# probabilists/zuko

Hardware: AMD Instinct MI355X
Metric: log_prob samples/sec, NSF d=64 K=8 bins=8 batch=2^20 (higher is better)
Workload: dtype f32; 1 GPU; NSF(features=64, context=0, transforms=8, bins=8, hidden=[256]*3) log_prob, batch=2^20 per GPU, x~N(0,1), seed-0 init; batch_per_gpu=1048576, global_batch=1048576, parallelism=batch-sharded x1, one RCCL all-reduce of the scalar NLL

## Files before the change

### zuko_amd/csrc/fused_ar_half_impl.h

```cpp
#pragma once
#include "fused_ar_split_impl.h"

#ifndef ARH_LOOK
#define ARH_LOOK 1
#endif
#ifndef ARH_RELU_INT
#define ARH_RELU_INT 0
#endif
#ifndef ARH_EPI_PINNED
#define ARH_EPI_PINNED 1
#endif
#ifndef ARH_DESCALE_PK
#define ARH_DESCALE_PK 1
#endif
#ifndef ARH_PREFETCH
#define ARH_PREFETCH 1
#endif

namespace zk {

typedef _Float16 f16x8 __attribute__((ext_vector_type(8)));

struct ArhB {
  f16x8 h, l;
};

__device__ __forceinline__ void arh_scale(float& amax, float& s, float& inv_s) {
  amax = fmaxf(amax, __shfl_xor(amax, 16, 64));
  amax = fmaxf(amax, __shfl_xor(amax, 32, 64));
  int e = __builtin_amdgcn_frexp_expf(amax);
  int ea = 15 - e;
  ea = ea > 90 ? 90 : (ea < -90 ? -90 : ea);
  s = __builtin_amdgcn_ldexpf(1.0f, ea);
  inv_s = __builtin_amdgcn_ldexpf(1.0f, -ea);
}

#define ARH_AMAX_OVERFLOW (65520.f * 0x1p90f)

typedef unsigned arh_u32x4 __attribute__((ext_vector_type(4)));
typedef float arh_f32x2 __attribute__((ext_vector_type(2)));

__device__ __forceinline__ void arh_split(const f32x4& lo, const f32x4& hi, float s, ArhB& b) {
  if (ARX_ABL == 6) {
    b.h = __builtin_bit_cast(f16x8, lo); b.l = __builtin_bit_cast(f16x8, hi);
    return;
  }
#if ARH_EPI_PINNED
  const float nz = -0.f;
  arh_u32x4 h, l;
#pragma unroll
  for (int e = 0; e < 4; ++e) asm("v_fma_mixlo_f16 %0, %1, %2, %3" : "=v"(h[e]) : "v"(e < 2 ? lo[2 * e] : hi[2 * e - 4]), "v"(s), "s"(nz));
#pragma unroll
  for (int e = 0; e < 4; ++e) asm("v_fma_mixhi_f16 %0, %1, %2, %3" : "+v"(h[e]) : "v"(e < 2 ? lo[2 * e + 1] : hi[2 * e - 3]), "v"(s), "s"(nz));
#pragma unroll
  for (int e = 0; e < 4; ++e) asm("v_fma_mixlo_f16 %0, %1, %2, -%3 op_sel:[0,0,0] op_sel_hi:[0,0,1]" : "=v"(l[e]) : "v"(e < 2 ? lo[2 * e] : hi[2 * e - 4]), "v"(s), "v"(h[e]));
#pragma unroll
  for (int e = 0; e < 4; ++e) asm("v_fma_mixhi_f16 %0, %1, %2, -%3 op_sel:[0,0,1] op_sel_hi:[0,0,1]" : "+v"(l[e]) : "v"(e < 2 ? lo[2 * e + 1] : hi[2 * e - 3]), "v"(s), "v"(h[e]));
  b.h = __builtin_bit_cast(f16x8, h); b.l = __builtin_bit_cast(f16x8, l);
  return;
#endif
#pragma unroll
  for (int e = 0; e < 8; ++e) {
    const float v = (e < 4 ? lo[e] : hi[e - 4]) * s;
    const _Float16 h = (_Float16)v;
    const float r = v - (float)h;
    b.h[e] = h;
    b.l[e] = (_Float16)r;
  }
}

#define ARH_MFMA(A, B, C) C = __builtin_amdgcn_mfma_f32_16x16x32_f16(__builtin_bit_cast(f16x8, A), B, C, 0, 0, 0)
__device__ __forceinline__ void arh_block(const f32x4 (&a)[2], const ArhB& b, f32x4& c) {
  if (ARX_ABL == 2) {
    asm volatile("" ::"v"(a[0]), "v"(a[1]));
    return;
  }
  ARH_MFMA(a[1], b.h, c);
  ARH_MFMA(a[0], b.l, c);
  ARH_MFMA(a[0], b.h, c);
}

__device__ __forceinline__ void arh_touch(f32x4& v) { asm volatile("" : "+v"(v)); }
template <int N> __device__ __forceinline__ void arh_settle(f32x4& a0, f32x4& a1) { asm volatile("s_waitcnt lgkmcnt(%2)" : "+v"(a0), "+v"(a1) : "n"(N)); }
template <int N> __device__ __forceinline__ void arh_settle(f32x4& a0, f32x4& a1, f32x4& a2) { asm volatile("s_waitcnt lgkmcnt(%3)" : "+v"(a0), "+v"(a1), "+v"(a2) : "n"(N)); }

template <int WAVES, int CH, int NR> struct ArhRing : ArRingS<WAVES, CH, NR> {
  typedef ArRingS<WAVES, CH, NR> B;
  template <int XV> __device__ __forceinline__ void advance_x() {
    asm volatile("s_waitcnt vmcnt(%0) lgkmcnt(0)" ::"n"((NR - 2) * B::PER + XV) : "memory");
    if (ARX_ABL != 4) __builtin_amdgcn_s_barrier();
    asm volatile("" ::: "memory");
    this->issue();
    this->slot = (this->slot + 1 == NR) ? 0 : this->slot + 1;
    this->cur_off = this->lds_off + (unsigned)(this->slot * CH * AR_TF * 4 + this->lane * 16);
  }
  template <int S, int XV = 0> __device__ __forceinline__ f32x4 read() {
    if constexpr (XV != 0 && S % CH == 0) {
      advance_x<XV>();
      f32x4 v;
      if (ARX_ABL == 5) {
        asm volatile("v_mov_b32 %0, %1" : "=v"(v[0]) : "v"(this->cur_off));
        v[1] = v[2] = v[3] = v[0];
        return v;
      }
      asm volatile("ds_read_b128 %0, %1 offset:%2" : "=v"(v) : "v"(this->cur_off), "n"((S % CH) * AR_TF * 4));
      return v;
    } else {
      return B::template read<S>();
    }
  }
};

template <int WAVES, int CH, int IMAGES, int BPOS, bool FLOW = false> struct ArhRing4 {
  static constexpr int NR = 4, PER = CH / WAVES, PIVOT = PER > 4 ? 4 : 0, CHB = CH * AR_TF * 4, NCH = (IMAGES + CH - 1) / CH;
  static_assert(PER * WAVES == CH && PER <= 6 && BPOS % 2 == 0 && BPOS >= 2 * (ARH_LOOK + 1) && BPOS + 1 < CH && CH % 2 == 0 && IMAGES % 2 == 0, "ring geometry");
  static constexpr int trigger(int c) {
    const int last = (IMAGES < (c + 1) * CH ? IMAGES : (c + 1) * CH) - 1;
    return c * CH + BPOS + 1 < last ? c * CH + BPOS + 1 : last;
  }
  static constexpr int first_trigger_from(int pos) {
    for (int c = 0; c < NCH; ++c)
      if (trigger(c) >= pos) return trigger(c);
    return -1;
  }
  const char* gsrc;
  char* ldst;
  unsigned goff, gend;
  unsigned fill_off;
  unsigned read_off;
  unsigned lane_off;
  unsigned lane16;
  unsigned cur_off;
  bool rows_in_flight;
  const char* bias_src;
  char* bias_dst;
  int bias_n, wave_id;
  __device__ __forceinline__ void bias_request() {
    for (int p = wave_id; p < bias_n; p += WAVES)
      __builtin_amdgcn_global_load_lds((const __attribute__((address_space(1))) void*)(bias_src + p * 1024 + (size_t)lane16), (__attribute__((address_space(3))) void*)(bias_dst + p * 1024), 16, 0, 0);
  }
  __device__ __forceinline__ void start(float* lds, const float* stream, int n_chunks, int wave, int lane) {
    const int b0 = wave * PER + PIVOT;
    gsrc = reinterpret_cast<const char*>(stream + b0 * AR_TF);
    ldst = reinterpret_cast<char*>(lds + b0 * AR_TF);
    goff = 0; gend = (unsigned)n_chunks * CHB; fill_off = 0;
    lane16 = (unsigned)lane * 16;
    lane_off = (unsigned)(size_t)((__attribute__((address_space(3))) float*)lds) + lane16;
    if constexpr (FLOW) { wave_id = wave; rows_in_flight = false; bias_n = 0; }
#pragma unroll
    for (int i = 0; i < NR - 1; ++i) issue();
    read_off = (NR - 1) * CHB;
    cur_off = lane_off;
  }
  template <int I> __device__ __forceinline__ void dma(const char* g, char* l) {
    if constexpr (I < PER) {
      __builtin_amdgcn_global_load_lds((const __attribute__((address_space(1))) void*)g, (__attribute__((address_space(3))) void*)l, 16, (I - PIVOT) * AR_TF * 4, 0);
      dma<I + 1>(g, l);
    }
  }
  __device__ __forceinline__ void issue() {
    asm volatile("" : "+v"(lane16));
    if (ARX_ABL != 1) dma<0>(gsrc + goff + (size_t)lane16, ldst + fill_off);
    goff = (goff + CHB == gend) ? 0 : goff + CHB;
    fill_off = (fill_off + CHB == NR * CHB) ? 0 : fill_off + CHB;
  }
  template <int XV, bool DRAIN> __device__ __forceinline__ void wait() {
    if constexpr (DRAIN) asm volatile("s_waitcnt vmcnt(%0) lgkmcnt(0)" ::"n"(XV) : "memory");
    else asm volatile("s_waitcnt vmcnt(%0)" ::"n"(XV) : "memory");
  }
  template <int XV, bool DRAIN> __device__ __forceinline__ void boundary() {
    if constexpr (FLOW && XV != 0) {
      if (rows_in_flight) wait<XV, DRAIN>();
      else wait<0, DRAIN>();
    } else {
      wait<XV, DRAIN>();
    }
    if (ARX_ABL != 4) __builtin_amdgcn_s_barrier();
    asm volatile("" ::: "memory");
    issue();
    asm volatile("" ::: "memory");
  }
  template <int S, int XV = 0> __device__ __forceinline__ f32x4 read() {
    static_assert(S >= 0 && S < IMAGES, "stream position");
    if constexpr (S % CH == 0) {
      read_off = (read_off + CHB == NR * CHB) ? 0 : read_off + CHB;
      cur_off = lane_off + read_off;
    }
    f32x4 v;
    if (ARX_ABL == 5) {
      asm volatile("v_mov_b32 %0, %1" : "=v"(v[0]) : "v"(cur_off));
      v[1] = v[2] = v[3] = v[0];
    } else {
      asm volatile("ds_read_b128 %0, %1 offset:%2" : "=v"(v) : "v"(cur_off), "n"((S % CH) * AR_TF * 4));
    }
    if constexpr (S == trigger(S / CH)) boundary<XV, (S % CH != BPOS + 1)>();
    if constexpr (FLOW && NCH >= 2) {
      if constexpr (S == trigger(NCH - 2)) bias_request();
    }
    return v;
  }
};

template <class S, int L, bool ALT> constexpr int arh_ip(int s) {
  if constexpr (ALT) return S::B_IP_ALT[s];
  else return ArxPat<S>::ip(L, s);
}
template <class S, int L, class Ring, bool ALT = false> __device__ __forceinline__ void arh_hidden(Ring& ring, const float* bias_q, const ArhB (&in)[S::TMAX / 2], f32x4 (&out)[S::TMAX], float d) {
  typedef ArxPat<S> P;
  constexpr int NB = S::NB[L], BASE = S::BASE[L], HTL = S::HT[L];
  ars_for<HTL>([&](auto t_) ARS_ALWAYS_INLINE {
    constexpr int t = t_;
    if constexpr (!P::tile_has_blocks(L, t)) out[t] = *reinterpret_cast<const f32x4*>(bias_q + t * 16);
  });
  if constexpr (NB > 0) {
    constexpr int LOOK = ARH_LOOK < NB ? ARH_LOOK : NB;
    f32x4 a[LOOK + 1][2];
    f32x4 bs;
    f32x4 acc;
    const unsigned bias_addr = arx_lds_addr(bias_q);
    ars_for<LOOK>([&](auto b_) ARS_ALWAYS_INLINE {
      constexpr int b = b_;
      ars_for<2>([&](auto p) ARS_ALWAYS_INLINE { a[b][p] = ring.template read<BASE + 2 * b + decltype(p)::value>(); });
    });
    ars_for<NB>([&](auto s_) ARS_ALWAYS_INLINE {
      constexpr int s = s_, ot = P::ot(L, s), cur = s % (LOOK + 1);
      constexpr int ip = arh_ip<S, L, ALT>(s);
      constexpr bool first_of_tile = (s == 0 || P::ot(L, s - 1) != ot), last_of_tile = (s + 1 == NB || P::ot(L, s + 1) != ot);
      if constexpr (first_of_tile) acc = f32x4{0.f, 0.f, 0.f, 0.f};
      if constexpr (last_of_tile) bs = arx_lds_raw<ot * 64>(bias_addr);
      if constexpr (s + LOOK < NB) {
        constexpr int nx = (s + LOOK) % (LOOK + 1);
        ars_for<2>([&](auto p) ARS_ALWAYS_INLINE { a[nx][p] = ring.template read<BASE + 2 * (s + LOOK) + decltype(p)::value>(); });
      }
      constexpr int ahead = (s + LOOK < NB ? LOOK : NB - 1 - s);
      if constexpr (last_of_tile) arh_settle<(s + LOOK < NB ? 2 : 0)>(a[cur][0], a[cur][1], bs);
      else arh_settle<2 * ahead>(a[cur][0], a[cur][1]);
      if (ARX_FENCE) __builtin_amdgcn_sched_barrier(0);
      arh_block(a[cur], in[ip], acc);
      if (ARX_FENCE) __builtin_amdgcn_sched_barrier(0);
      if constexpr (last_of_tile) {
        if (ARH_DESCALE_PK) {
#pragma unroll
          for (int r = 0; r < 4; r += 2) {
            const arh_f32x2 o = __builtin_elementwise_fma(arh_f32x2{acc[r], acc[r + 1]}, arh_f32x2{d, d}, arh_f32x2{bs[r], bs[r + 1]});
            out[ot][r] = o[0]; out[ot][r + 1] = o[1];
          }
        } else {
#pragma unroll
          for (int r = 0; r < 4; ++r) out[ot][r] = __builtin_fmaf(acc[r], d, bs[r]);
        }
      }
    });
  }
}

template <class S, int L, class Ring, bool HAS_ALT = false> __device__ __forceinline__ void arh_hidden_stack(Ring& ring, const float* bias_lds, int q, ArhB (&in)[S::TMAX / 2], f32x4 (&out)[S::TMAX], const float* wd,
                                                                                                         float& inv_s, float& poison, bool alt = false) {
  if constexpr (L < S::NH) {
    if constexpr (HAS_ALT && L == 0) {
      static_assert(S::BASE[0] == 0, "B_IP_ALT lists the first layer's blocks");
      if (alt) arh_hidden<S, L, Ring, true>(ring, bias_lds + L * S::BIAS_STRIDE + 4 * q, in, out, wd[L] * inv_s);
      else arh_hidden<S, L, Ring>(ring, bias_lds + L * S::BIAS_STRIDE + 4 * q, in, out, wd[L] * inv_s);
    } else {
      arh_hidden<S, L, Ring>(ring, bias_lds + L * S::BIAS_STRIDE + 4 * q, in, out, wd[L] * inv_s);
    }
    constexpr int HTL = S::HT[L];
    float amax = 0.f;
    if constexpr (S::ACT == 1 && ARH_EPI_PINNED) {
#pragma unroll
      for (int t = 0; t < HTL; ++t)
#pragma unroll
        for (int r = 0; r < 4; r += 2) {
          asm("v_max_f32 %0, 0, %0" : "+v"(out[t][r]));
          asm("v_max_f32 %0, 0, %0" : "+v"(out[t][r + 1]));
          asm("v_max3_f32 %0, %0, %1, %2" : "+v"(amax) : "v"(out[t][r]), "v"(out[t][r + 1]));
        }
    } else if constexpr (S::ACT == 1) {
#pragma unroll
      for (int t = 0; t < HTL; ++t)
#pragma unroll
        for (int r = 0; r < 4; ++r) {
          if (ARH_RELU_INT) out[t][r] = __builtin_bit_cast(float, max(__builtin_bit_cast(int, out[t][r]), 0));
          else out[t][r] = out[t][r] < 0.f ? 0.f : out[t][r];
          amax = fmaxf(amax, out[t][r]);
        }
    } else {
      ar_activate<S::ACT, HTL>(out, out);
#pragma unroll
      for (int t = 0; t < HTL; ++t)
#pragma unroll
        for (int r = 0; r < 4; ++r) amax = fmaxf(amax, fabsf(out[t][r]));
    }
    float s;
    arh_scale(amax, s, inv_s);
    if constexpr (S::ACT == 1 && ARH_EPI_PINNED) {
      if (!(amax < ARH_AMAX_OVERFLOW)) poison = __builtin_nanf("");
    }
    const f32x4 zero = {0.f, 0.f, 0.f, 0.f};
#pragma unroll
    for (int p = 0; p < (HTL + 1) / 2; ++p) arh_split(out[2 * p], 2 * p + 1 < HTL ? out[2 * p + 1] : zero, s, in[p]);
    arh_hidden_stack<S, L + 1, Ring, HAS_ALT>(ring, bias_lds, q, in, out, wd, inv_s, poison, alt);
  }
}

template <typename Uni> __device__ __forceinline__ void arh_flow_epilogue(float (&p)[4 * Uni::NT], const ArArgs& a, const int (&fid)[Uni::FPL], const float (&xin)[Uni::FPL], float poison, float* xr,
                                                                          const float* base, int D, bool term, float& lacc) {
  constexpr int FPL = Uni::FPL, TOTAL = Uni::TOTAL;
#pragma unroll
  for (int fi = 0; fi < FPL; ++fi) Uni::template poison<false>(p, fi * TOTAL, poison);
  auto ld = [&](int i) { return p[i]; };
#pragma unroll
  for (int fi = 0; fi < FPL; ++fi) {
    const int f = fid[fi];
    if (f >= 0) {
      float yv, lj;
      Uni::fwd(ld, fi * TOTAL, a, xin[fi], yv, lj);
      lacc += lj;
      if (term) {
        const float df = yv - base[f];
        lacc += __builtin_fmaf(-(df * df), base[D + f], base[2 * D + f]);
      } else {
        xr[f] = yv;
      }
    }
  }
}

template <class S, typename Uni, bool DIAG, bool TERM, bool FLOW, class Ring, class XReq, class Fids>
__device__ __forceinline__ void arh_pass(const ArArgs& a, Ring& ring, XReq& x_request, f32x4 (&xnext)[S::NIT], float* bias_lds, const Fids& fids, float* xr, const float* base, const ArLane& ln,
                                         int64_t tile, const float* wd, bool first, bool last, bool term, float& total, bool alt = false) {
  constexpr bool RING4 = S::NR == 4;
  static_assert(!FLOW || (RING4 && S::XLDS && S::DIN == S::D && !DIAG && !TERM), "flow pass: four-slot ring, rows in LDS, no context columns");
  constexpr int NT = Uni::NT, FPL = Uni::FPL, WAVES = S::WAVES;
  constexpr int NG = S::NG;
  constexpr int NSTEP = S::GOFF[NG];
  constexpr bool XLDS = S::XLDS;
  const int wave = ln.wave, j = ln.j, q = ln.q;
  const float* bias_last = bias_lds + S::NH * S::BIAS_STRIDE;
  const unsigned bias_last_addr = arx_lds_addr(bias_last + 4 * q);
  if constexpr (FLOW) {
    asm volatile("" ::: "memory");
    __builtin_amdgcn_wave_barrier();
  }
  const int64_t n = tile * (16 * WAVES) + wave * 16 + j;
  const bool live = n < a.N;
  const int64_t nc = live ? n : a.N - 1;
  const float* xrow = a.x + nc * a.ldx;

  ArhB in[S::TMAX / 2];
  f32x4 out[S::TMAX];
  float poison;
  float inv_s;
  {
    f32x4 xin[S::NIT + 1];
#pragma unroll
    for (int it = 0; it < S::NIT; ++it) {
      f32x4 v = {0.f, 0.f, 0.f, 0.f};
      if constexpr (FLOW) {
        if ((it + 1) * 16 <= S::DIN || it * 16 + 4 * q < S::DIN) v = *reinterpret_cast<const f32x4*>(xr + it * 16 + 4 * q);
      } else if (ARH_PREFETCH) {
        if ((it + 1) * 16 <= S::DIN || it * 16 + 4 * q < S::DIN) v = xnext[it];
      } else {
        if ((it + 1) * 16 <= S::DIN || it * 16 + 4 * q < S::DIN) v = *reinterpret_cast<const f32x4*>(xrow + it * 16 + 4 * q);
      }
      xin[it] = v;
    }
    xin[S::NIT] = f32x4{0.f, 0.f, 0.f, 0.f};
    poison = ar_poison_of<S::NIT>(xin);
    float amax = 0.f;
#pragma unroll
    for (int it = 0; it < S::NIT; ++it)
#pragma unroll
      for (int r = 0; r < 4; ++r) amax = fmaxf(amax, fabsf(xin[it][r]));
    if constexpr (XLDS && !FLOW) ar_rows_in<S::D>(xr, q, xin);
    float s;
    arh_scale(amax, s, inv_s);
    if constexpr (S::ACT == 1 && ARH_EPI_PINNED) {
      if (!(amax < ARH_AMAX_OVERFLOW)) poison = __builtin_nanf("");
    }
#pragma unroll
    for (int p = 0; p < (S::NIT + 1) / 2; ++p) arh_split(xin[2 * p], xin[2 * p + 1], s, in[p]);
  }

  float ladj_in = 0.f;
  if constexpr (!FLOW) {
    if (ARH_PREFETCH && a.ladj && a.accumulate && live && q == 0) ladj_in = a.ladj[n];
  }

  if constexpr (FLOW) arh_hidden_stack<S, 0, Ring, S::FLOW_ALT>(ring, bias_lds, q, in, out, wd, inv_s, poison, alt);
  else arh_hidden_stack<S, 0, Ring>(ring, bias_lds, q, in, out, wd, inv_s, poison);

  const float dl = wd[S::NH] * inv_s;
  float lacc = 0.f;
  constexpr int NBL = NSTEP * NT;
  constexpr int LOOKL = ARH_LOOK < NBL ? ARH_LOOK : NBL;
  f32x4 w[LOOKL + 1][2];
  constexpr int XPOS = []() constexpr {
    if constexpr (!ARH_PREFETCH) return -1;
    else if constexpr (RING4) return Ring::first_trigger_from(S::LAST_BASE);
    else return (S::LAST_BASE + S::CH - 1) / S::CH * S::CH;
  }();
  if constexpr (FLOW) {
    asm volatile("" ::: "memory");
    if (last) {
      x_request(tile + gridDim.x < a.n_tiles ? tile + gridDim.x : tile, xnext);
    } else {
#pragma unroll
      for (int it = 0; it < S::NIT; ++it) asm("" : "=v"(xnext[it]));
    }
    ring.rows_in_flight = last;
    asm volatile("" ::: "memory");
  } else if (ARH_PREFETCH) {
    asm volatile("" ::: "memory");
    x_request(tile + gridDim.x < a.n_tiles ? tile + gridDim.x : tile, xnext);
    asm volatile("" ::: "memory");
  }
#define ARH_READ_LAST(POS) ring.template read<(POS), ((POS) == XPOS ? S::NIT : 0)>()
  ars_for<LOOKL>([&](auto b_) ARS_ALWAYS_INLINE {
    constexpr int b = b_;
    ars_for<2>([&](auto p) ARS_ALWAYS_INLINE { w[b][p] = ARH_READ_LAST(S::LAST_BASE + 2 * b + decltype(p)::value); });
  });
  ars_for<NG>([&](auto g_) ARS_ALWAYS_INLINE {
    constexpr int g = g_, ST0 = S::GOFF[g], GN = S::GOFF[g + 1] - S::GOFF[g];
    int fid[FPL];
    float xin[FPL];
    fids.template fetch<XLDS>(g, xr, xrow, fid, xin);
    float bv[3 * FPL];
    if constexpr (TERM && !FLOW) fids.fetch_base(fid, base, S::D, bv);
    f32x4 acc[NT], bs[NT];
    if constexpr (GN == 0) {
      const float* bg = bias_last + (g * NT) * 16 + 4 * q;
      ars_for<NT>([&](auto t) ARS_ALWAYS_INLINE { bs[t] = *reinterpret_cast<const f32x4*>(bg + t * 16); });
    }
    ars_for<NT>([&](auto t) ARS_ALWAYS_INLINE { acc[t] = f32x4{0.f, 0.f, 0.f, 0.f}; });
    ars_for<GN>([&](auto i_) ARS_ALWAYS_INLINE {
      constexpr int st = ST0 + decltype(i_)::value, ip = S::G_IP[st];
      ars_for<NT>([&](auto t_) ARS_ALWAYS_INLINE {
        constexpr int t = t_, blk = st * NT + t, cur = blk % (LOOKL + 1);
        constexpr bool last_of_group = (decltype(i_)::value == GN - 1 && t == NT - 1);
        if constexpr (last_of_group) {
          ars_for<NT>([&](auto u) ARS_ALWAYS_INLINE { bs[u] = arx_lds_raw<(g * NT + decltype(u)::value) * 64>(bias_last_addr); });
        }
        if constexpr (blk + LOOKL < NBL) {
          constexpr int nx = (blk + LOOKL) % (LOOKL + 1);
          ars_for<2>([&](auto p) ARS_ALWAYS_INLINE { w[nx][p] = ARH_READ_LAST(S::LAST_BASE + 2 * (blk + LOOKL) + decltype(p)::value); });
        }
        constexpr int ahead = (blk + LOOKL < NBL ? LOOKL : NBL - 1 - blk);
        if constexpr (last_of_group) arh_settle<(blk + LOOKL < NBL ? 2 : 0)>(w[cur][0], w[cur][1]);
        else arh_settle<2 * ahead>(w[cur][0], w[cur][1]);
        if constexpr (last_of_group) {
#pragma unroll
          for (int u = 0; u < NT; ++u) arh_touch(bs[u]);
        }
        if (ARX_FENCE) __builtin_amdgcn_sched_barrier(0);
        arh_block(w[cur], in[ip], acc[t]);
        if (ARX_FENCE) __builtin_amdgcn_sched_barrier(0);
      });
    });
    float p[4 * NT];
    ars_for<NT>([&](auto t) ARS_ALWAYS_INLINE {
#pragma unroll
      for (int r = 0; r < 4; ++r) {
        p[4 * t + r] = __builtin_fmaf(acc[t][r], dl, bs[t][r]);
        if (ARH_POISON_ONE) asm("" : "+v"(p[4 * t + r]));
      }
    });
    if constexpr (FLOW) arh_flow_epilogue<Uni>(p, a, fid, xin, poison, xr, base, S::D, last && term, lacc);
    else ar_uni_epilogue<Uni, DIAG, XLDS, true, TERM>(p, a, fid, xin, poison, xr, n, live, S::D, lacc, bv);
  });
#undef ARH_READ_LAST
  if constexpr (FLOW) {
    lacc += __shfl_xor(lacc, 16, 64);
    lacc += __shfl_xor(lacc, 32, 64);
    total = first ? lacc : total + lacc;
    if (last) {
      if (live && q == 0) a.ladj[n] = total;
      if (!term) ar_rows_out<S::D>(xr, q, a.y + n * a.ldy, live);
    }
    return;
  }
  if (ARH_PREFETCH) ar_ladj_store<true>(a, lacc, n, live, q, ladj_in);
  if constexpr (XLDS && !TERM) ar_rows_out<S::D>(xr, q, a.y + n * a.ldy, live);
  if (!ARH_PREFETCH) ar_ladj_store(a, lacc, n, live, q);
}

template <class S, typename Uni, bool DIAG, bool TERM> __device__ __forceinline__ void arh_body(const ArArgs& a) {
  constexpr bool RING4 = S::NR == 4;
  typedef std::conditional_t<RING4, ArhRing4<S::WAVES, S::CH, S::IMAGES, S::BPOS>, ArhRing<S::WAVES, S::CH, S::NR>> Ring;
  static_assert(S::WAVES == 8 && (S::NR == 3 || S::NR == 4) && S::TMAX <= 16 && S::TMAX % 2 == 0 && S::OCC == 2, "two-part split kernels: widths <= 256, two wavefronts per SIMD");
  constexpr int NT = Uni::NT, FPL = Uni::FPL, WAVES = S::WAVES;
  constexpr int NG = S::NG;
  constexpr int NSTEP = S::GOFF[NG];
  static_assert(S::IMAGES == S::LAST_BASE + 2 * NSTEP * NT && (S::IMAGES + S::CH - 1) / S::CH == S::NCHUNK, "stream length");
  const ArLane ln;
  const int tid = ln.tid, lane = ln.lane, wave = ln.wave, j = ln.j, q = ln.q;

  Ring ring;
  if constexpr (RING4) {
    ring.start(ars_lds, a.stream, a.n_chunks, wave, lane);
  } else {
    ring.lds = ars_lds; ring.stream = a.stream; ring.n_chunks = a.n_chunks; ring.wave = wave; ring.lane = lane;
    ring.load_chunk = 0; ring.load_slot = 0;
#pragma unroll
    for (int i = 0; i < S::NR - 1; ++i) ring.issue();
    ring.slot = S::NR - 1;
    ring.lds_off = (unsigned)(size_t)((__attribute__((address_space(3))) float*)ars_lds);
    ring.cur_off = ring.lds_off;
  }

  auto x_request = [&](int64_t tile, f32x4 (&xv)[S::NIT]) ARS_ALWAYS_INLINE {
    const int64_t n = tile * (16 * WAVES) + wave * 16 + j;
    const float* row = a.x + (n < a.N ? n : a.N - 1) * a.ldx;
#pragma unroll
    for (int it = 0; it < S::NIT; ++it) {
      const int col = it * 16 + 4 * q;
      xv[it] = *reinterpret_cast<const f32x4*>(row + ((it + 1) * 16 <= S::DIN || col < S::DIN ? col : S::DIN - 4));
    }
  };
  f32x4 xnext[S::NIT];
  if (ARH_PREFETCH) x_request(blockIdx.x, xnext);

  float* const bias_lds = ars_lds + S::NR * S::CH * AR_TF;
  int* const fmap_lds = ArLds::fmap(bias_lds, a.bias_floats);
  float* const xr = ArLds::row(fmap_lds, wave, j, a.xs);
  float* const base = ArLds::base(fmap_lds, NG * 4 * FPL);
  if constexpr (TERM) ArLds::stage_base<64 * WAVES>(a, tid, base, S::D);
  ArLds::stage<64 * WAVES>(a, tid, bias_lds, fmap_lds, NG * 4 * FPL);
  const ArFids<NG, FPL, (NG * FPL <= 32)> fids(fmap_lds, q);

  float unused = 0.f;
  for (int64_t tile = blockIdx.x; tile < a.n_tiles; tile += gridDim.x)
    arh_pass<S, Uni, DIAG, TERM, false>(a, ring, x_request, xnext, bias_lds, fids, xr, base, ln, tile, a.wdescale, true, true, TERM, unused);
  asm volatile("s_waitcnt vmcnt(0)" ::: "memory");
}

template <class S, typename Uni, bool DIAG = false> __global__ __launch_bounds__(64 * S::WAVES, S::OCC) void arh_kernel(ArArgs a) { arh_body<S, Uni, DIAG, false>(a); }
template <class S, typename Uni> __global__ __launch_bounds__(64 * S::WAVES, S::OCC) void arht_kernel(ArArgs a) { arh_body<S, Uni, false, true>(a); }

template <class S, typename Uni> static int arh_launch(const ArArgs* in, int abi, int args_bytes, int train, void* stream) {
  if (abi != ARS_ABI || args_bytes != (int)sizeof(ArArgs)) return ZK_EINVAL;
  ArArgs a = *in;
  if (train || a.D != S::D || a.DIN != S::DIN || a.L != S::NH + 1 || a.act != S::ACT || a.sched || a.NG != S::NG || a.n_chunks != S::NCHUNK || a.l1rev) return ZK_EINVAL;
  for (int l = 0; l <= S::NH; ++l)
    if (!(a.wdescale[l] > 0.f) || !(a.wdescale[l] < __builtin_inff())) return ZK_EINVAL;
  a.n_tiles = (a.N + 16 * S::WAVES - 1) / (16 * S::WAVES);
  a.xs = ((S::D + 3) / 4) * 4 + 4;
  const bool term = a.base_loc != nullptr;
  if (term && (!a.base_scale || !a.ladj || a.bin_out || a.knots_out || !ArLds::base_fits(S::NG * 4 * Uni::FPL, S::D))) return ZK_EINVAL;
  const bool vec_ok = (S::D % 4 == 0) && (term || ((a.ldy % 4 == 0) && ((uintptr_t)a.y % 16 == 0)));
  if (S::XLDS != 0 && !vec_ok) return ZK_EINVAL;
  a.xlds = S::XLDS;
  const int lds = ArLds::bytes(S::NR * S::CH * AR_TF, a.bias_floats, S::XLDS ? S::WAVES : 0, a.xs);
  if (lds > 160 * 1024) return ZK_EINVAL;
  const void* fn = nullptr;
  if ((a.bin_out != nullptr) != (a.knots_out != nullptr)) return ZK_EINVAL;
  if (term) {
    fn = (const void*)arht_kernel<S, Uni>;
  } else if (a.bin_out) {
    if constexpr (Uni::NKNOT > 1) fn = (const void*)arh_kernel<S, Uni, true>;
  } else {
    fn = (const void*)arh_kernel<S, Uni, false>;
  }
  if (!fn) return ZK_EINVAL;
  return ar_launch_dyn_lds(fn, 256, 64 * S::WAVES, lds, a, stream);
}

template <class S, typename Uni> __device__ __forceinline__ void arhf_body(const ArArgs& a, const ArhFlow& f) {
  typedef ArhRing4<S::WAVES, S::CH, S::IMAGES, S::BPOS, true> Ring;
  static_assert(S::WAVES == 8 && S::NR == 4 && S::TMAX <= 16 && S::TMAX % 2 == 0 && S::OCC == 2 && S::NCHUNK >= 2, "flow kernel: the four-slot two-part geometry, two chunks or more per pass");
  constexpr int NT = Uni::NT, FPL = Uni::FPL, WAVES = S::WAVES, NG = S::NG, NFM = NG * 4 * FPL;
  static_assert(S::IMAGES == S::LAST_BASE + 2 * S::GOFF[NG] * NT && (S::IMAGES + S::CH - 1) / S::CH == S::NCHUNK, "stream length");
  const ArLane ln;
  const int tid = ln.tid, lane = ln.lane, wave = ln.wave, j = ln.j, q = ln.q;

  Ring ring;
  ring.start(ars_lds, a.stream, f.T * a.n_chunks, wave, lane);
  auto x_request = [&](int64_t tile, f32x4 (&xv)[S::NIT]) ARS_ALWAYS_INLINE {
    const int64_t n = tile * (16 * WAVES) + wave * 16 + j;
    const float* row = a.x + (n < a.N ? n : a.N - 1) * a.ldx;
#pragma unroll
    for (int it = 0; it < S::NIT; ++it) {
      const int col = it * 16 + 4 * q;
      xv[it] = *reinterpret_cast<const f32x4*>(row + ((it + 1) * 16 <= S::DIN || col < S::DIN ? col : S::DIN - 4));
    }
  };
  f32x4 xnext[S::NIT];
  x_request(blockIdx.x, xnext);

  float* const bias_lds = ars_lds + S::NR * S::CH * AR_TF;
  int* const fmap_lds = ArLds::fmap(bias_lds, 2 * f.bias_stride);
  float* const xr = ArLds::row(fmap_lds, wave, j, a.xs);
  float* const base = ArLds::base(fmap_lds, f.n_fmaps * NFM);
  if (f.term) ArLds::stage_base<64 * WAVES>(a, tid, base, S::D);
  for (int i = tid; i < a.bias_floats; i += 64 * WAVES) bias_lds[i] = f.bias[i];
  for (int i = tid; i < f.n_fmaps * NFM; i += 64 * WAVES) fmap_lds[i] = f.featmap[i];
  __syncthreads();
  ring.bias_n = f.bias_stride / 256;
  const __attribute__((address_space(4))) float* const table = (const __attribute__((address_space(4))) float*)f.table;

  int buf = 0;
  for (int64_t tile = blockIdx.x; tile < a.n_tiles; tile += gridDim.x) {
    ar_rows_in<S::D>(xr, q, xnext);
    float total = 0.f;
#pragma unroll 1
    for (int t = 0; t < f.T; ++t) {
      float wd[4];
#pragma unroll
      for (int l = 0; l < 4; ++l) wd[l] = table[t * 8 + l];
      const int fm = __builtin_bit_cast(int, table[t * 8 + 4]);
      const bool alt = __builtin_bit_cast(int, table[t * 8 + 5]) != 0;
      const int tn = t + 1 == f.T ? 0 : t + 1;
      ring.bias_src = reinterpret_cast<const char*>(f.bias + (size_t)tn * f.bias_stride);
      ring.bias_dst = reinterpret_cast<char*>(bias_lds + (buf ^ 1) * f.bias_stride);
      const ArFids<NG, FPL, (NG * FPL <= 32)> fids(fmap_lds + fm * NFM, q);
      arh_pass<S, Uni, false, false, true>(a, ring, x_request, xnext, bias_lds + buf * f.bias_stride, fids, xr, base, ln, tile, wd, t == 0, t + 1 == f.T, f.term != 0, total, alt);
      buf ^= 1;
    }
  }
  asm volatile("s_waitcnt vmcnt(0)" ::: "memory");
}

template <class S, typename Uni> __global__ __launch_bounds__(64 * S::WAVES, S::OCC) void arhf_kernel(ArArgs a, ArhFlow f) { arhf_body<S, Uni>(a, f); }

template <class S, typename Uni> static int arhf_launch(const ArArgs* in, const ArhFlow* fin, int abi, int args_bytes, int flow_bytes, void* stream) {
  if (abi != ARS_ABI || args_bytes != (int)sizeof(ArArgs) || flow_bytes != (int)sizeof(ArhFlow)) return ZK_EINVAL;
  if constexpr (S::NR != 4 || !S::XLDS || S::DIN != S::D || S::D % 4 != 0 || S::NCHUNK < 2) {
    return ZK_EINVAL;
  } else {
    ArArgs a = *in;
    ArhFlow f = *fin;
    if (a.D != S::D || a.DIN != S::DIN || a.L != S::NH + 1 || a.act != S::ACT || a.sched || a.NG != S::NG || a.n_chunks != S::NCHUNK || a.l1rev) return ZK_EINVAL;
    if (f.T < 1 || f.T > 64 || f.n_fmaps < 1 || f.n_fmaps > f.T || f.bias_stride % 256 || f.bias_stride < a.bias_floats || !f.bias || !f.featmap || !f.table) return ZK_EINVAL;
    if (!a.x || !a.stream || !a.ladj || a.accumulate || a.bin_out || a.knots_out) return ZK_EINVAL;
    a.n_tiles = (a.N + 16 * S::WAVES - 1) / (16 * S::WAVES);
    a.xs = ((S::D + 3) / 4) * 4 + 4;
    f.term = a.base_loc != nullptr;
    if (f.term ? !a.base_scale : (!a.y || a.ldy % 4 != 0 || (uintptr_t)a.y % 16 != 0)) return ZK_EINVAL;
    if (f.n_fmaps * S::NG * 4 * Uni::FPL + (f.term ? 3 * S::D : 0) > ArLds::FMAP_WORDS) return ZK_EINVAL;
    a.xlds = 1;
    const int lds = ArLds::bytes(S::NR * S::CH * AR_TF, 2 * f.bias_stride, S::WAVES, a.xs);
    if (lds > 160 * 1024) return ZK_EINVAL;
    const void* fn = (const void*)arhf_kernel<S, Uni>;
    hipError_t e = grant_dyn_lds(fn, lds);
    if (e != hipSuccess) return (int)e;
    const unsigned grid = (unsigned)(a.n_tiles < 256 ? a.n_tiles : 256);
    void* kargs[] = {&a, &f};
    e = hipLaunchKernel(fn, dim3(grid), dim3(64 * S::WAVES), kargs, lds, (hipStream_t)stream);
    if (e != hipSuccess) return (int)e;
    return ZK_LAUNCH_CHECK();
  }
}

}
```

Measured before the change: 75.92 million samples/s.

## Hand-schedule MFMA blocks and split in inline asm, fuse ReLU-max per tile

Replaces the three-MFMA split-precision block with one inline-asm sequence that includes the LDS waitcnt. The first block of each tile uses a zero C operand, which removes the explicit accumulator zeroing, and explicit s_nop padding covers MFMA result hazards. The fp16 hi/lo split becomes a single asm block with early-clobber outputs. The ReLU and amax reduction are moved into each tile's epilogue, using four partial maxima that are joined at the end. The aim is to cut scheduling slack and instruction overhead, at the cost of fragile hand-managed hazards and extra register pressure.

```diff
diff --git a/zuko_amd/csrc/fused_ar_half_impl.h b/zuko_amd/csrc/fused_ar_half_impl.h
--- a/zuko_amd/csrc/fused_ar_half_impl.h
+++ b/zuko_amd/csrc/fused_ar_half_impl.h
@@ -16,6 +16,12 @@
 #ifndef ARH_PREFETCH
 #define ARH_PREFETCH 1
 #endif
+#ifndef ARH_BLOCK_ASM
+#define ARH_BLOCK_ASM 1
+#endif
+#ifndef ARH_EPI_TILE
+#define ARH_EPI_TILE 1
+#endif
 
 namespace zk {
 
@@ -47,16 +53,18 @@
   }
 #if ARH_EPI_PINNED
   const float nz = -0.f;
-  arh_u32x4 h, l;
-#pragma unroll
-  for (int e = 0; e < 4; ++e) asm("v_fma_mixlo_f16 %0, %1, %2, %3" : "=v"(h[e]) : "v"(e < 2 ? lo[2 * e] : hi[2 * e - 4]), "v"(s), "s"(nz));
-#pragma unroll
-  for (int e = 0; e < 4; ++e) asm("v_fma_mixhi_f16 %0, %1, %2, %3" : "+v"(h[e]) : "v"(e < 2 ? lo[2 * e + 1] : hi[2 * e - 3]), "v"(s), "s"(nz));
-#pragma unroll
-  for (int e = 0; e < 4; ++e) asm("v_fma_mixlo_f16 %0, %1, %2, -%3 op_sel:[0,0,0] op_sel_hi:[0,0,1]" : "=v"(l[e]) : "v"(e < 2 ? lo[2 * e] : hi[2 * e - 4]), "v"(s), "v"(h[e]));
-#pragma unroll
-  for (int e = 0; e < 4; ++e) asm("v_fma_mixhi_f16 %0, %1, %2, -%3 op_sel:[0,0,1] op_sel_hi:[0,0,1]" : "+v"(l[e]) : "v"(e < 2 ? lo[2 * e + 1] : hi[2 * e - 3]), "v"(s), "v"(h[e]));
-  b.h = __builtin_bit_cast(f16x8, h); b.l = __builtin_bit_cast(f16x8, l);
+  unsigned h0, h1, h2, h3, l0, l1, l2, l3;
+#define ARH_SPLIT_H(OP, H, V) "v_fma_mix" OP "_f16 %[" H "], %[" V "], %[s], %[nz]\n\t"
+#define ARH_SPLIT_L(OP, SEL, L, H, V) "v_fma_mix" OP "_f16 %[" L "], %[" V "], %[s], -%[" H "] op_sel:[0,0," SEL "] op_sel_hi:[0,0,1]\n\t"
+  asm(ARH_SPLIT_H("lo", "h0", "v0") ARH_SPLIT_H("lo", "h1", "v2") ARH_SPLIT_H("lo", "h2", "v4") ARH_SPLIT_H("lo", "h3", "v6")
+      ARH_SPLIT_H("hi", "h0", "v1") ARH_SPLIT_H("hi", "h1", "v3") ARH_SPLIT_H("hi", "h2", "v5") ARH_SPLIT_H("hi", "h3", "v7")
+      ARH_SPLIT_L("lo", "0", "l0", "h0", "v0") ARH_SPLIT_L("lo", "0", "l1", "h1", "v2") ARH_SPLIT_L("lo", "0", "l2", "h2", "v4") ARH_SPLIT_L("lo", "0", "l3", "h3", "v6")
+      ARH_SPLIT_L("hi", "1", "l0", "h0", "v1") ARH_SPLIT_L("hi", "1", "l1", "h1", "v3") ARH_SPLIT_L("hi", "1", "l2", "h2", "v5") ARH_SPLIT_L("hi", "1", "l3", "h3", "v7")
+      : [h0] "=&v"(h0), [h1] "=&v"(h1), [h2] "=&v"(h2), [h3] "=&v"(h3), [l0] "=&v"(l0), [l1] "=&v"(l1), [l2] "=&v"(l2), [l3] "=&v"(l3)
+      : [v0] "v"(lo[0]), [v1] "v"(lo[1]), [v2] "v"(lo[2]), [v3] "v"(lo[3]), [v4] "v"(hi[0]), [v5] "v"(hi[1]), [v6] "v"(hi[2]), [v7] "v"(hi[3]), [s] "v"(s), [nz] "s"(nz));
+#undef ARH_SPLIT_H
+#undef ARH_SPLIT_L
+  b.h = __builtin_bit_cast(f16x8, arh_u32x4{h0, h1, h2, h3}); b.l = __builtin_bit_cast(f16x8, arh_u32x4{l0, l1, l2, l3});
   return;
 #endif
 #pragma unroll
@@ -83,6 +91,46 @@
 __device__ __forceinline__ void arh_touch(f32x4& v) { asm volatile("" : "+v"(v)); }
 template <int N> __device__ __forceinline__ void arh_settle(f32x4& a0, f32x4& a1) { asm volatile("s_waitcnt lgkmcnt(%2)" : "+v"(a0), "+v"(a1) : "n"(N)); }
 template <int N> __device__ __forceinline__ void arh_settle(f32x4& a0, f32x4& a1, f32x4& a2) { asm volatile("s_waitcnt lgkmcnt(%3)" : "+v"(a0), "+v"(a1), "+v"(a2) : "n"(N)); }
+
+constexpr bool ARH_BLK = ARH_BLOCK_ASM && ARX_ABL != 2;
+#define ARH_BLK_ASM(C0, COUT, POST, BSOUT)                                                                  \
+  asm volatile("v_mfma_f32_16x16x32_f16 %[c], %[al], %[bh], " C0 "\n\t"                                     \
+               "v_mfma_f32_16x16x32_f16 %[c], %[ah], %[bl], %[c]\n\t"                                       \
+               "v_mfma_f32_16x16x32_f16 %[c], %[ah], %[bh], %[c]" POST                                      \
+               : [c] COUT(c) ARH_BLK_BS##BSOUT                                                              \
+               : [ah] "v"(a[0]), [al] "v"(a[1]), [bh] "v"(b.h), [bl] "v"(b.l))
+#define ARH_BLK_BS0
+#define ARH_BLK_BS1 , "+v"(bs)
+template <int N, bool FIRST, bool PAD, bool TILE> __device__ __forceinline__ void arh_wait_block(f32x4 (&a)[2], const ArhB& b, f32x4& c, f32x4& bs) {
+  static_assert(N >= 0 && N < 16, "lgkmcnt is a four-bit field");
+  if constexpr (PAD) asm volatile("s_nop 0");
+  __builtin_amdgcn_s_waitcnt(0xC07F | (N << 8));
+  if (ARX_FENCE) __builtin_amdgcn_sched_barrier(0);
+  if constexpr (FIRST && TILE) ARH_BLK_ASM("0", "=&v", "\n\ts_nop 11", 1);
+  else if constexpr (FIRST) ARH_BLK_ASM("0", "=&v", "", 0);
+  else if constexpr (TILE) ARH_BLK_ASM("%[c]", "+v", "\n\ts_nop 11", 1);
+  else ARH_BLK_ASM("%[c]", "+v", "", 0);
+  if (ARX_FENCE) __builtin_amdgcn_sched_barrier(0);
+}
+#undef ARH_BLK_ASM
+#undef ARH_BLK_BS0
+#undef ARH_BLK_BS1
+template <int NT> __device__ __forceinline__ void arh_acc_ready(f32x4 (&acc)[NT]) {
+  asm volatile("s_nop 11" : "+v"(acc[NT - 1]));
+#pragma unroll
+  for (int t = 0; t + 1 < NT; ++t) arh_touch(acc[t]);
+}
+
+__device__ __forceinline__ void arh_relu_max(f32x4& o, float (&pm)[4], int t) {
+#pragma unroll
+  for (int r = 0; r < 4; r += 2)
+    asm("v_max_f32 %0, 0, %0\n\tv_max_f32 %1, 0, %1\n\tv_max3_f32 %2, %2, %0, %1" : "+v"(o[r]), "+v"(o[r + 1]), "+v"(pm[(2 * t + r / 2) % 4]));
+}
+__device__ __forceinline__ float arh_join_max(const float (&pm)[4]) {
+  float amax;
+  asm("v_max_f32 %0, %1, %2\n\tv_max3_f32 %0, %0, %3, %4" : "=&v"(amax) : "v"(pm[0]), "v"(pm[1]), "v"(pm[2]), "v"(pm[3]));
+  return amax;
+}
 
 template <int WAVES, int CH, int NR> struct ArhRing : ArRingS<WAVES, CH, NR> {
   typedef ArRingS<WAVES, CH, NR> B;
@@ -205,12 +253,16 @@
   if constexpr (ALT) return S::B_IP_ALT[s];
   else return ArxPat<S>::ip(L, s);
 }
-template <class S, int L, class Ring, bool ALT = false> __device__ __forceinline__ void arh_hidden(Ring& ring, const float* bias_q, const ArhB (&in)[S::TMAX / 2], f32x4 (&out)[S::TMAX], float d) {
+template <class S> constexpr bool ARH_EPI = S::ACT == 1 && ARH_EPI_PINNED && ARH_EPI_TILE;
+template <class S, int L, class Ring, bool ALT = false> __device__ __forceinline__ void arh_hidden(Ring& ring, const float* bias_q, const ArhB (&in)[S::TMAX / 2], f32x4 (&out)[S::TMAX], float d, float (&pm)[4]) {
   typedef ArxPat<S> P;
   constexpr int NB = S::NB[L], BASE = S::BASE[L], HTL = S::HT[L];
   ars_for<HTL>([&](auto t_) ARS_ALWAYS_INLINE {
     constexpr int t = t_;
-    if constexpr (!P::tile_has_blocks(L, t)) out[t] = *reinterpret_cast<const f32x4*>(bias_q + t * 16);
+    if constexpr (!P::tile_has_blocks(L, t)) {
+      out[t] = *reinterpret_cast<const f32x4*>(bias_q + t * 16);
+      if constexpr (ARH_EPI<S>) arh_relu_max(out[t], pm, t);
+    }
   });
   if constexpr (NB > 0) {
     constexpr int LOOK = ARH_LOOK < NB ? ARH_LOOK : NB;
@@ -226,18 +278,22 @@
       constexpr int s = s_, ot = P::ot(L, s), cur = s % (LOOK + 1);
       constexpr int ip = arh_ip<S, L, ALT>(s);
       constexpr bool first_of_tile = (s == 0 || P::ot(L, s - 1) != ot), last_of_tile = (s + 1 == NB || P::ot(L, s + 1) != ot);
-      if constexpr (first_of_tile) acc = f32x4{0.f, 0.f, 0.f, 0.f};
+      if constexpr (first_of_tile && !ARH_BLK) acc = f32x4{0.f, 0.f, 0.f, 0.f};
       if constexpr (last_of_tile) bs = arx_lds_raw<ot * 64>(bias_addr);
       if constexpr (s + LOOK < NB) {
         constexpr int nx = (s + LOOK) % (LOOK + 1);
         ars_for<2>([&](auto p) ARS_ALWAYS_INLINE { a[nx][p] = ring.template read<BASE + 2 * (s + LOOK) + decltype(p)::value>(); });
       }
       constexpr int ahead = (s + LOOK < NB ? LOOK : NB - 1 - s);
-      if constexpr (last_of_tile) arh_settle<(s + LOOK < NB ? 2 : 0)>(a[cur][0], a[cur][1], bs);
-      else arh_settle<2 * ahead>(a[cur][0], a[cur][1]);
-      if (ARX_FENCE) __builtin_amdgcn_sched_barrier(0);
-      arh_block(a[cur], in[ip], acc);
-      if (ARX_FENCE) __builtin_amdgcn_sched_barrier(0);
+      if constexpr (ARH_BLK) {
+        arh_wait_block<(last_of_tile ? (s + LOOK < NB ? 2 : 0) : 2 * ahead), first_of_tile, s == 0, last_of_tile>(a[cur], in[ip], acc, bs);
+      } else {
+        if constexpr (last_of_tile) arh_settle<(s + LOOK < NB ? 2 : 0)>(a[cur][0], a[cur][1], bs);
+        else arh_settle<2 * ahead>(a[cur][0], a[cur][1]);
+        if (ARX_FENCE) __builtin_amdgcn_sched_barrier(0);
+        arh_block(a[cur], in[ip], acc);
+        if (ARX_FENCE) __builtin_amdgcn_sched_barrier(0);
+      }
       if constexpr (last_of_tile) {
         if (ARH_DESCALE_PK) {
 #pragma unroll
@@ -249,6 +305,7 @@
 #pragma unroll
           for (int r = 0; r < 4; ++r) out[ot][r] = __builtin_fmaf(acc[r], d, bs[r]);
         }
+        if constexpr (ARH_EPI<S>) arh_relu_max(out[ot], pm, ot);
       }
     });
   }
@@ -257,24 +314,22 @@
 template <class S, int L, class Ring, bool HAS_ALT = false> __device__ __forceinline__ void arh_hidden_stack(Ring& ring, const float* bias_lds, int q, ArhB (&in)[S::TMAX / 2], f32x4 (&out)[S::TMAX], const float* wd,
                                                                                                          float& inv_s, float& poison, bool alt = false) {
   if constexpr (L < S::NH) {
+    float pm[4] = {0.f, 0.f, 0.f, 0.f};
     if constexpr (HAS_ALT && L == 0) {
       static_assert(S::BASE[0] == 0, "B_IP_ALT lists the first layer's blocks");
-      if (alt) arh_hidden<S, L, Ring, true>(ring, bias_lds + L * S::BIAS_STRIDE + 4 * q, in, out, wd[L] * inv_s);
-      else arh_hidden<S, L, Ring>(ring, bias_lds + L * S::BIAS_STRIDE + 4 * q, in, out, wd[L] * inv_s);
+      if (alt) arh_hidden<S, L, Ring, true>(ring, bias_lds + L * S::BIAS_STRIDE + 4 * q, in, out, wd[L] * inv_s, pm);
+      else arh_hidden<S, L, Ring>(ring, bias_lds + L * S::BIAS_STRIDE + 4 * q, in, out, wd[L] * inv_s, pm);
     } else {
-      arh_hidden<S, L, Ring>(ring, bias_lds + L * S::BIAS_STRIDE + 4 * q, in, out, wd[L] * inv_s);
+      arh_hidden<S, L, Ring>(ring, bias_lds + L * S::BIAS_STRIDE + 4 * q, in, out, wd[L] * inv_s, pm);
     }
     constexpr int HTL = S::HT[L];
     float amax = 0.f;
     if constexpr (S::ACT == 1 && ARH_EPI_PINNED) {
-#pragma unroll
-      for (int t = 0; t < HTL; ++t)
-#pragma unroll
-        for (int r = 0; r < 4; r += 2) {
-          asm("v_max_f32 %0, 0, %0" : "+v"(out[t][r]));
-          asm("v_max_f32 %0, 0, %0" : "+v"(out[t][r + 1]));
-          asm("v_max3_f32 %0, %0, %1, %2" : "+v"(amax) : "v"(out[t][r]), "v"(out[t][r + 1]));
-        }
+      if constexpr (!ARH_EPI_TILE) {
+#pragma unroll
+        for (int t = 0; t < HTL; ++t) arh_relu_max(out[t], pm, t);
+      }
+      amax = arh_join_max(pm);
     } else if constexpr (S::ACT == 1) {
 #pragma unroll
       for (int t = 0; t < HTL; ++t)
@@ -432,7 +487,7 @@
       const float* bg = bias_last + (g * NT) * 16 + 4 * q;
       ars_for<NT>([&](auto t) ARS_ALWAYS_INLINE { bs[t] = *reinterpret_cast<const f32x4*>(bg + t * 16); });
     }
-    ars_for<NT>([&](auto t) ARS_ALWAYS_INLINE { acc[t] = f32x4{0.f, 0.f, 0.f, 0.f}; });
+    if constexpr (GN == 0 || !ARH_BLK) ars_for<NT>([&](auto t) ARS_ALWAYS_INLINE { acc[t] = f32x4{0.f, 0.f, 0.f, 0.f}; });
     ars_for<GN>([&](auto i_) ARS_ALWAYS_INLINE {
       constexpr int st = ST0 + decltype(i_)::value, ip = S::G_IP[st];
       ars_for<NT>([&](auto t_) ARS_ALWAYS_INLINE {
@@ -446,15 +501,24 @@
           ars_for<2>([&](auto p) ARS_ALWAYS_INLINE { w[nx][p] = ARH_READ_LAST(S::LAST_BASE + 2 * (blk + LOOKL) + decltype(p)::value); });
         }
         constexpr int ahead = (blk + LOOKL < NBL ? LOOKL : NBL - 1 - blk);
-        if constexpr (last_of_group) arh_settle<(blk + LOOKL < NBL ? 2 : 0)>(w[cur][0], w[cur][1]);
-        else arh_settle<2 * ahead>(w[cur][0], w[cur][1]);
-        if constexpr (last_of_group) {
-#pragma unroll
-          for (int u = 0; u < NT; ++u) arh_touch(bs[u]);
+        if constexpr (ARH_BLK) {
+          arh_wait_block<(last_of_group ? (blk + LOOKL < NBL ? 2 : 0) : 2 * ahead), decltype(i_)::value == 0, blk == 0, false>(w[cur], in[ip], acc[t], bs[0]);
+          if constexpr (last_of_group) {
+#pragma unroll
+            for (int u = 0; u < NT; ++u) arh_touch(bs[u]);
+            arh_acc_ready<NT>(acc);
+          }
+        } else {
+          if constexpr (last_of_group) arh_settle<(blk + LOOKL < NBL ? 2 : 0)>(w[cur][0], w[cur][1]);
+          else arh_settle<2 * ahead>(w[cur][0], w[cur][1]);
+          if constexpr (last_of_group) {
+#pragma unroll
+            for (int u = 0; u < NT; ++u) arh_touch(bs[u]);
+          }
+          if (ARX_FENCE) __builtin_amdgcn_sched_barrier(0);
+          arh_block(w[cur], in[ip], acc[t]);
+          if (ARX_FENCE) __builtin_amdgcn_sched_barrier(0);
         }
-        if (ARX_FENCE) __builtin_amdgcn_sched_barrier(0);
-        arh_block(w[cur], in[ip], acc[t]);
-        if (ARX_FENCE) __builtin_amdgcn_sched_barrier(0);
       });
     });
     float p[4 * NT];
```

Result: faster. 77.06 million samples/s, median of 6 (+1.5%).
